# YeLyuUT/VOSDetectron

Hardware: AMD Instinct MI355X
Metric: frames/sec @1333x800 e2e_mask_rcnn_R-50-FPN, 1/2/4/8 MI355X; RoIAlign HBM GB/s (higher is better)
Workload: dtype fp32; 1 GPU; e2e_mask_rcnn_R-50-FPN_1x inference, 64 synthetic 800x1333 frames per GPU per step: blob, body, RPN, proposals, box head, class NMS, mask head -> class-selected masks (segm_results paste/RLE excluded, SURVEY 8d); frames_per_gpu_step=64, global_batch=64, layout=nhwc, gather_bytes_per_rank=0, launch=hipGraph replay per step

## Files before the change

### include/vosdet.h

```cpp
#ifndef VOSDET_H_
#define VOSDET_H_

#include <stddef.h>
#include <stdint.h>

#ifdef __cplusplus
extern "C" {
#endif

#define VD_MAX_LEVELS 5

enum {
    VD_OK = 0,
    VD_ERR_ARG = 1,
    VD_ERR_SHAPE = 2,
    VD_ERR_LAUNCH = 3,
    VD_ERR_WORKSPACE = 4
};

enum { VD_LAYOUT_NCHW = 0, VD_LAYOUT_NHWC = 1 };

#define VD_COUNT_SELECT_FAILED (-1)
#define VD_COUNT_PREV_BOXES (-2)

// ... 65 lines not shown
                        const float *bias, int relu, float *Y, void *stream);

int vd_conv3x3_wino_weight(const float *w, int Cout, int Cin, float *U, void *stream);
int vd_conv3x3_wino_bias_act(const float *X, int N, int H, int W, int C, const float *U,
                             int Cout, const float *bias, int relu, float *Y, void *stream);

int vd_conv3x3_wino4_weight(const float *w, int Cout, int Cin, float *U, void *stream);
int vd_conv3x3_wino4_bias_act(const float *X, int N, int H, int W, int C, const float *U,
                              int Cout, const float *bias, int relu, float *Y, void *stream);
int vd_conv3x3_wino4_mosaic_bias_act(const float *X, int N, int H, int W, int C, const float *U,
                                     int Cout, const float *bias, int relu, float *Y,
                                     void *stream);
int vd_conv3x3_wino4_rows_bias_act(const float *X, int N, int H, int W, int C, const float *U,
                                   int Cout, const float *bias, int relu, float *Y,
                                   void *stream);
int vd_conv3x3_wino4_grouped_bias_act(const float *X, int N, int H, int W, int C,
                                      const float *U, int groups, const float *bias, int relu,
                                      float *Y, int rows, void *stream);
int vd_conv3x3_wino4_dilated2_bias_act(const float *X, int N, int H, int W, int C,
                                       const float *U, int Cout, const float *bias, int relu,
                                       float *Y, int layout, void *stream);
int vd_conv3x3_wino4_grid_bias_act(const float *X, int N, int H, int W, int C, const float *U,
                                   int Cout, const float *bias, int relu, float *Y,
                                   void *stream);

int vd_conv3x3_wino_seg_bias_act(const float *X, int H, int W, int C, const float *U, int Cout,
                                 const float *bias, int relu, int seg_h, float *Y, void *stream);

int vd_conv3x3_wino_mosaic_bias_act(const float *X, int R, int H, int W, int C, const float *U,
                                    int Cout, const float *bias, int relu, float *Y, void *stream);
// ... 185 lines not shown
```

### vosdetectron_amd/_lib.py

```python
from __future__ import annotations

import ctypes
import os
import threading

_HERE = os.path.dirname(os.path.abspath(__file__))
LIB_PATH = os.path.join(_HERE, "libvosdet.so")
if os.environ.get("VOSDET_RESEARCH_LIB"):
    LIB_PATH = os.environ["VOSDET_RESEARCH_LIB"]
GEMM_PLANS = os.path.join(_HERE, "gemm_plans.txt")
os.environ.setdefault("VOSDET_GEMM_PLANS", GEMM_PLANS)

VD_OK, VD_ERR_ARG, VD_ERR_SHAPE, VD_ERR_LAUNCH, VD_ERR_WORKSPACE = range(5)
VD_LAYOUT_NCHW, VD_LAYOUT_NHWC = 0, 1
VD_MAX_LEVELS = 5
VD_ACT_NONE, VD_ACT_RELU, VD_ACT_SIGMOID, VD_ACT_TANH = range(4)

_lock = threading.Lock()
_lib = None


class VdFeatLevel(ctypes.Structure):
    _fields_ = [("data", ctypes.c_void_p), ("H", ctypes.c_int), ("W", ctypes.c_int),
                ("spatial_scale", ctypes.c_float)]
# ... 29 lines not shown
    "vd_gemm_dual_bias_act": (_I, [_P, _I, _P, _I, _I, _P, _I, _P, _I, _P, _P]),
    "vd_gemm_split3_weight_size": (_S, [_I, _I]),
    "vd_mask_head_upconv_logits": (_I, [_P, _I, _I, _P, _P, _P, _P, _P, _I, _P, _P]),
    "vd_gemm_split3_weight": (_I, [_P, _I, _I, _P, _P]),
    "vd_gemm_split3_bias_act": (_I, [_P, _I, _I, _P, _I, _P, _P, _I, _P, _P, _I, _I, _I, _I,
                                    _I, _P, _I, _P]),
    "vd_fpn_lateral_weight": (_I, [_P, _I, _I, _P, _P]),
    "vd_fpn_lateral_topdown": (_I, [_P, _L, _I, _P, _I, _P, _P, _I, _I, _P, _P]),
    "vd_conv3x3_bias_act": (_I, [_P, _I, _I, _I, _I, _P, _I, _P, _I, _P, _P]),
    "vd_conv3x3_wino_weight": (_I, [_P, _I, _I, _P, _P]),
    "vd_conv3x3_wino_bias_act": (_I, [_P, _I, _I, _I, _I, _P, _I, _P, _I, _P, _P]),
    "vd_conv3x3_wino4_weight": (_I, [_P, _I, _I, _P, _P]),
    "vd_conv3x3_wino4_bias_act": (_I, [_P, _I, _I, _I, _I, _P, _I, _P, _I, _P, _P]),
    "vd_conv3x3_wino4_mosaic_bias_act": (_I, [_P, _I, _I, _I, _I, _P, _I, _P, _I, _P, _P]),
    "vd_conv3x3_wino4_rows_bias_act": (_I, [_P, _I, _I, _I, _I, _P, _I, _P, _I, _P, _P]),
    "vd_conv3x3_wino4_grid_bias_act": (_I, [_P, _I, _I, _I, _I, _P, _I, _P, _I, _P, _P]),
    "vd_conv3x3_wino4_dilated2_bias_act": (_I, [_P, _I, _I, _I, _I, _P, _I, _P, _I, _P, _I,
                                                _P]),
    "vd_conv3x3_wino4_grouped_bias_act": (_I, [_P, _I, _I, _I, _I, _P, _I, _P, _I, _P, _I,
                                               _P]),
    "vd_conv3x3_wino_seg_bias_act": (_I, [_P, _I, _I, _I, _P, _I, _P, _I, _I, _P, _P]),
    "vd_conv3x3_wino_mosaic_bias_act": (_I, [_P, _I, _I, _I, _I, _P, _I, _P, _I, _P, _P]),
    "vd_roi_align_legacy_forward": (_I, [_I, _I, _F, _P, _I, _I, _I, _I, _P, _I, _P, _P]),
    "vd_roi_pool_forward": (_I, [_I, _I, _F, _P, _I, _I, _I, _I, _P, _I, _P, _P, _P]),
    "vd_roi_pool_backward": (_I, [_P, _P, _L, _P, _P]),
    "vd_roi_crop_forward": (_I, [_P, _I, _I, _I, _I, _P, _I, _I, _I, _P, _P]),
    "vd_nms_workspace_size": (_S, [_I]),
    "vd_nms": (_I, [_P, _I, _I, _F, _P, _P, _P, _S, _P]),
    "vd_map_rois_to_fpn_levels": (_I, [_P, _I, _I, _I, _I, _I, _F, _F, _P, _P]),
    "vd_mask_rois": (_I, [_P, _P, _P, _I, _I, _P, _I, _I, _I, _I, _F, _F, _P, _P, _P, _P, _P]),
# ... 77 lines not shown
```

### vosdetectron_amd/csrc/capi.cpp

```cpp
#include <hip/hip_runtime.h>

#include "vosdet_internal.hpp"

using namespace vd;

#define VD_STREAM(s) reinterpret_cast<hipStream_t>(s)

extern "C" {

int vd_version(void) { return 1; }

const char *vd_status_string(int status) {
    switch (status) {
        case VD_OK: return "ok";
        case VD_ERR_ARG: return "invalid argument";
        case VD_ERR_SHAPE: return "unsupported shape";
        case VD_ERR_LAUNCH: return "kernel launch failed";
        case VD_ERR_WORKSPACE: return "workspace too small";
        default: return "unknown status";
    }
}

static bool bad_feat(const void *p, int B, int C, int H, int W) {
    return !p || B < 1 || C < 1 || H < 1 || W < 1;
// ... 163 lines not shown

int vd_conv3x3_wino4_mosaic_bias_act(const float *X, int N, int H, int W, int C, const float *U,
                                     int Cout, const float *bias, int relu, float *Y,
                                     void *stream) {
    if (N < 0 || H < 1 || W < 1 || C < 1 || Cout < 1 || !U || !Y || (N > 0 && !X))
        return VD_ERR_ARG;
    return launch_conv3x3_wino4(X, N, H, W, C, U, Cout, bias, relu, Y, VD_STREAM(stream), 1);
}

int vd_conv3x3_wino4_rows_bias_act(const float *X, int N, int H, int W, int C, const float *U,
                                   int Cout, const float *bias, int relu, float *Y,
                                   void *stream) {
    if (N < 0 || H < 1 || W < 1 || C < 1 || Cout < 1 || !U || !Y || (N > 0 && !X))
        return VD_ERR_ARG;
    return launch_conv3x3_wino4(X, N, H, W, C, U, Cout, bias, relu, Y, VD_STREAM(stream), 2);
}

int vd_conv3x3_wino4_grouped_bias_act(const float *X, int N, int H, int W, int C,
                                      const float *U, int groups, const float *bias, int relu,
                                      float *Y, int rows, void *stream) {
    if (N < 0 || H < 1 || W < 1 || C < 1 || groups < 1 || !U || !Y || (N > 0 && !X))
        return VD_ERR_ARG;
    return launch_conv3x3_wino4(X, N, H, W, C, U, C, bias, relu, Y, VD_STREAM(stream),
                                rows ? 2 : 0, groups);
}

int vd_conv3x3_wino4_dilated2_bias_act(const float *X, int N, int H, int W, int C,
                                       const float *U, int Cout, const float *bias, int relu,
                                       float *Y, int layout, void *stream) {
    if (N < 0 || H < 2 || W < 2 || (H & 1) || (W & 1) || C < 1 || Cout < 1 || !U || !Y ||
// ... 522 lines not shown
```

### vosdetectron_amd/csrc/conv3x3_wino4.hip

```cpp
#include <stdlib.h>

#include "common.hpp"
#include "vosdet_internal.hpp"

namespace vd {

namespace {

typedef float f4v __attribute__((ext_vector_type(4)));
typedef float f2v __attribute__((ext_vector_type(2)));

constexpr int k4Co = 64;
constexpr int k4KC = 8;
constexpr int k4Threads = 512;
constexpr int k4TR = 4, k4TC = 8;
constexpr int k4PR = 4 * k4TR + 2;
constexpr int k4PC = 4 * k4TC + 2;
constexpr int k4RP = 84;
constexpr int k4PSlots = 1536;
constexpr int k4PStageB = k4PSlots * 16;
constexpr int k4VStageB = 36 * 32 * k4KC * 4;
constexpr int k4ZeroF4 = 1024;
constexpr int k4LdsB = 2 * k4VStageB + 2 * k4PStageB + 6 * 256 * 4;

// ... 49 lines not shown
    y[5] = w4_pfma(4.f, x[1], w4_pfma(-5.f, x[3], x[5]));
}

__device__ __forceinline__ void w4_at6(const float (&m)[6], float (&y)[4]) {
    const float s12 = m[1] + m[2], d12 = m[1] - m[2], s34 = m[3] + m[4], d34 = m[3] - m[4];
    y[0] = m[0] + s12 + s34;
    y[1] = __builtin_fmaf(2.f, d34, d12);
    y[2] = __builtin_fmaf(4.f, s34, s12);
    y[3] = __builtin_fmaf(8.f, d34, d12) + m[5];
}

constexpr int kStampWg = 512, kStampCh0 = 8, kStampNch = 4;
__device__ unsigned long long g_wino4_stamps[kStampWg * 8 * kStampNch * 6];

template <bool RELU, int PROBE, bool ACC = false, int VD = 1, bool STAMP = false, bool IL = false,
          bool PK = false>
__global__ __launch_bounds__(k4Threads) void conv3x3_wino4_kernel(
    const float *__restrict__ X, int N, int H, int W, int C, const float *__restrict__ U,
    int Cout, const float *__restrict__ bias, float *__restrict__ Y, int tby, int tbx,
    int cb_per_xcd, int probe_hi, int mos, int gin) {
    __shared__ __attribute__((aligned(16))) char w4_lds[k4LdsB];
    float *const vst = reinterpret_cast<float *>(w4_lds);
    char *const pst = w4_lds + 2 * k4VStageB;
    const int tid = threadIdx.x, lane = tid & 63;
    const int wave = __builtin_amdgcn_readfirstlane(tid >> 6);
    const int ncb = Cout / k4Co;
    int cb, sp;
    if (cb_per_xcd) {
        const int xcd = blockIdx.x & 7;
        cb = xcd % ncb;
        sp = (blockIdx.x >> 3) * (8 / ncb) + xcd / ncb;
    } else {
        const int r8 = blockIdx.x % (8 * ncb);
        cb = r8 / 8;
        sp = (blockIdx.x / (8 * ncb)) * 8 + (r8 & 7);
    }
    const bool pair = mos == 1, oct = mos == 3, grid = (mos & 3) == 2;
    const int hp = (mos & 3) == 0 ? mos >> 2 : 0;
    const int gG = grid ? mos >> 2 : 0, gPh = H + 1, gPw = W + 1;
    if (sp >= (pair ? (N + 1) >> 1 : oct ? (N + 7) >> 3 : ((hp || grid) ? tby * tbx : N * tby * tbx))) return;
    const int n = pair ? 2 * sp : oct ? 8 * sp : ((hp || grid) ? 0 : sp / (tby * tbx));
    const int rem = (pair || oct) ? 0 : sp - n * tby * tbx;
    const int tyb = rem / tbx, txb = rem - (rem / tbx) * tbx;
    const int oy0 = 4 * k4TR * tyb, ox0 = 4 * k4TC * txb;
    const int iy0 = oy0 - 1, ix0 = ox0 - 1;
    const int nch = ((gin & 1) ? 64 : C) / k4KC;
    const uint32_t pbase = (uint32_t)(uintptr_t)pst;

    const bool pph = (gin & 2) != 0;
    const int pNr = N >> 2;
    const float *const Xn = X + (pph ? 0 : (int64_t)n * H * W * C) + ((gin & 1) ? 64 * cb : 0);
    auto px_off = [&](int m, int y, int x) -> int64_t {
        if (pph) {
            const int ab = m / pNr, nr = m - ab * pNr;
            return (((int64_t)nr * 2 * H + 2 * y + (ab >> 1)) * (2 * W) + 2 * x + (ab & 1));
        }
        return ((int64_t)m * H + y) * W + x;
    };
    uint32_t *const poff = reinterpret_cast<uint32_t *>(pst + 2 * k4PStageB) + tid;
    constexpr int kDW = ACC ? 8 : 4;
    constexpr int kDK = 24 / kDW;
    constexpr int kPS = ACC ? 512 : 256;
    const float *const zero = reinterpret_cast<const float *>(g_wino4_zero);
    const float *srcp[kDK];
#pragma unroll
    for (int k = 0; k < kDK; ++k) {
        if (!ACC && wave >= 4) break;
        const int s = 64 * (wave + kDW * k) + lane;
        const int R = s / k4RP, u = s - R * k4RP;
        const int m = u / 5, r5 = u - 5 * m;
        const int Cc = 2 * m + (r5 >> 1), hf = r5 & 1;
        const int y = iy0 + R, x = ix0 + Cc;
        const int gx = (grid && x >= 0) ? x / gPw : 0, gy = (grid && y >= 0) ? y / gPh : 0;
        const int cell = pair ? (x >> 4) : oct ? (x >> 3) : grid ? gx : 0;
        const int xm = pair ? (x & 15) : oct ? (x & 7) : grid ? x - gx * gPw : x;
        const int mr = (hp && y >= 0) ? y / hp : (oct && y >= 0) ? 4 * (y >> 3) : grid ? gG * gy : 0;
        const int ly = hp ? y - mr * hp : oct ? (y & 7) : grid ? y - gy * gPh : y;
        const bool ok = R < k4PR && r5 < 4 && Cc < k4PC && (unsigned)ly < (unsigned)H &&
                        y >= 0 && x >= 0 && (unsigned)xm < (unsigned)W && n + cell + mr < N &&
                        (!oct || (cell < 4 && mr < 8)) && (!grid || gx < gG);
        const int64_t po = pph ? px_off(n + cell + mr, ly, xm) : px_off(cell + mr, ly, xm);
        poff[kPS * k] = ok ? (uint32_t)(po * C + 4 * hf)
                           : 0x80000000u | (uint32_t)(4 * hf);
        srcp[k] = ok ? Xn + po * C + 4 * hf : zero + 4 * hf;
    }
    auto dma = [&](int ch, int stage) {
        if constexpr (ACC) {
#pragma unroll
            for (int k = 0; k < kDK; ++k)
                w4_dma_1k(srcp[k] + ch * k4KC,
                          pbase + (uint32_t)(stage * k4PStageB + (wave + kDW * k) * 1024));
            return;
        }
        uint32_t oo[kDK];
#pragma unroll
        for (int k = 0; k < kDK; ++k) oo[k] = poff[kPS * k];
#pragma unroll
        for (int k = 0; k < kDK; ++k) {
            const uint32_t o = oo[k];
            const float *src = (o & 0x80000000u) ? zero + (o & 7u) : Xn + o + ch * k4KC;
            if (ACC && ch < 0) src = zero;
            w4_dma_1k(src, pbase + (uint32_t)(stage * k4PStageB + (wave + kDW * k) * 1024));
        }
    };

    const int ttc = lane >> 3, tci = lane & 7;
    const float *const tread =
        reinterpret_cast<const float *>(pst) + ((4 * wave) * k4RP + 10 * ttc + (tci >> 2)) * 4 +
        (tci & 3);
    const int wtile_j = 8 * (wave & 1) + ttc;
    float *const twrite =
        ACC ? vst + (wave >> 1) * 128 + 32 * (tci >> 1) + ((2 * wtile_j + (tci & 1)) ^ (8 * (tci >> 1)))
            : vst + 64 * wave + lane;
    auto transform = [&](int stage) {
        const float *tp = tread + stage * (k4PStageB / 4);
        float *vp = twrite + stage * (k4VStageB / 4);
        if (PK) {
            f2v t[6][3];
#pragma unroll
            for (int c = 0; c < 6; c += 2) {
                f2v x[6], y[6];
#pragma unroll
                for (int r = 0; r < 6; ++r)
                    x[r] = f2v{tp[(r * k4RP + 2 * c + (c >> 1)) * 4],
                               tp[(r * k4RP + 2 * (c + 1) + ((c + 1) >> 1)) * 4]};
                w4_bt6v(x, y);
#pragma unroll
                for (int a = 0; a < 6; ++a) t[a][c >> 1] = y[a];
            }
#pragma unroll
            for (int a = 0; a < 6; a += 2) {
                f2v x[6], y[6];
#pragma unroll
                for (int c = 0; c < 6; ++c)
                    x[c] = f2v{t[a][c >> 1][c & 1], t[a + 1][c >> 1][c & 1]};
                w4_bt6v(x, y);
#pragma unroll
                for (int b = 0; b < 6; ++b) {
                    vp[(6 * a + b) * 256] = y[b][0];
                    vp[(6 * (a + 1) + b) * 256] = y[b][1];
                }
            }
            return;
        }
        float t[6][6];
#pragma unroll
        for (int c = 0; c < 6; ++c) {
            float x[6], y[6];
#pragma unroll
            for (int r = 0; r < 6; ++r) x[r] = tp[(r * k4RP + 2 * c + (c >> 1)) * 4];
            w4_bt6(x, y);
#pragma unroll
            for (int a = 0; a < 6; ++a) t[a][c] = y[a];
        }
#pragma unroll
        for (int a = 0; a < 6; ++a) {
            float y[6];
            w4_bt6(t[a], y);
#pragma unroll
            for (int b = 0; b < 6; ++b) vp[(6 * a + b) * 256] = y[b];
        }
    };

    const int tg = wave >> 2, cg = wave & 3;
    const int j = lane & 15, q = lane >> 4;
// ... 18 lines not shown
        w4_uload_asm(r, ursv, (uint32_t)uvoff,
                     (uint32_t)__builtin_amdgcn_readfirstlane((ch * 4 * 18 + pos) * 1024));
    };
    f4v acc[36];
#pragma unroll
    for (int p = 0; p < 36; ++p) acc[p] = f4v{0.f, 0.f, 0.f, 0.f};
    constexpr int kUR = 9;
    f4v u[kUR];
    auto mfma_chunk = [&](bool xon, int stage, int ch, int chn, int tstage) {
        const f2v *vp = vread + stage * (k4VStageB / 8);
        const float *tpi = tread + tstage * (k4PStageB / 4);
        float *vpw = twrite + tstage * (k4VStageB / 4);
        float xc[6], tt[6][6];
        if (IL && xon) {
#pragma unroll
            for (int r = 0; r < 6; ++r) xc[r] = tpi[(r * k4RP) * 4];
        }
        if (!IL && xon) {
            if (probe_hi & 2) asm volatile("s_setprio 1" ::: "memory");
            transform(tstage);
            if (probe_hi & 2) asm volatile("s_setprio 0" ::: "memory");
        }
        f2v vq[VD][2];
#pragma unroll
        for (int d = 0; d < VD; ++d) {
            vq[d][0] = vp[(2 * d) * 128];
            vq[d][1] = vp[(2 * d + 1) * 128];
        }
        f2v b0 = vq[0][0], b1 = vq[0][1];
#pragma unroll
        for (int pp = 0; pp < 18; ++pp) {
// ... 27 lines not shown
            } else if constexpr (!(PROBE & 8)) {
                if (pp + kUR < 18)
                    u[pp % kUR] = uload(ch, pp + kUR);
                else
                    u[pp % kUR] = uload(chn, pp + kUR - 18);
            }
            if constexpr (IL) {
                if (xon && pp < 6) {
                    float y[6];
                    w4_bt6(xc, y);
#pragma unroll
                    for (int a = 0; a < 6; ++a) tt[a][pp] = y[a];
                    if (pp < 5) {
                        const int c = pp + 1;
#pragma unroll
                        for (int r = 0; r < 6; ++r) xc[r] = tpi[(r * k4RP + 2 * c + (c >> 1)) * 4];
                    }
                } else if (xon && pp < 12) {
                    const int a = pp - 6;
                    float y[6];
                    w4_bt6(tt[a], y);
#pragma unroll
                    for (int b = 0; b < 6; ++b) vpw[(6 * a + b) * 256] = y[b];
                }
            }
            __builtin_amdgcn_sched_barrier(0);
            if (pp + VD < 18) {
                vq[pp % VD][0] = n0;
                vq[pp % VD][1] = n1;
            }
            if (pp < 17) {
// ... 53 lines not shown
    asm volatile("s_waitcnt vmcnt(0)" ::: "memory");
    __syncthreads();
    if (wave < 4) transform(0);
    if (wave < 4 && nch > 1) dma(1, 1);
    asm volatile("s_waitcnt vmcnt(0)" ::: "memory");
    __syncthreads();
    for (int ch = 0; ch < nch; ++ch) {
        const int sv = ch & 1;
        const int chn = ch + 1 < nch ? ch + 1 : ch;
        if (!(PROBE & 4) && wave < 4 && ch + 2 < nch) dma(ch + 2, sv);
        mfma_chunk(!(PROBE & 1) && wave < 4 && ch + 1 < nch, sv, ch, chn, sv ^ 1);
        asm volatile("s_waitcnt vmcnt(9)" ::: "memory");
        __syncthreads();
    }
    }
    asm volatile("s_waitcnt vmcnt(0)" ::: "memory");

    const int tile = 16 * tg + j, tr = tile >> 3, tc = tile & 7;
    const int co = cb * k4Co + 16 * cg + 4 * q;
    const float4 bv = bias ? *reinterpret_cast<const float4 *>(bias + co)
                           : make_float4(0.f, 0.f, 0.f, 0.f);
    float o[16][4];
#pragma unroll
    for (int r = 0; r < 4; ++r) {
        float tt[4][6];
#pragma unroll
        for (int b = 0; b < 6; ++b) {
            float m[6], y[4];
#pragma unroll
            for (int a = 0; a < 6; ++a) m[a] = acc[6 * a + b][r];
            w4_at6(m, y);
#pragma unroll
            for (int i = 0; i < 4; ++i) tt[i][b] = y[i];
        }
#pragma unroll
        for (int i = 0; i < 4; ++i) {
            float y[4];
            w4_at6(tt[i], y);
#pragma unroll
            for (int k = 0; k < 4; ++k) o[4 * i + k][r] = y[k];
        }
    }
#pragma unroll
    for (int i = 0; i < 4; ++i) {
        const int yv = oy0 + 4 * tr + i;
        const int gy = grid ? yv / gPh : 0;
        const int mr = hp ? yv / hp : oct ? 4 * (yv >> 3) : grid ? gG * gy : 0;
        const int yy = hp ? yv - mr * hp : oct ? (yv & 7) : grid ? yv - gy * gPh : yv;
        if (yy >= H || n + mr >= N) continue;
#pragma unroll
        for (int k = 0; k < 4; ++k) {
            const int xc = ox0 + 4 * tc + k;
            const int gx = grid ? xc / gPw : 0;
            const int ncell = pair ? n + (xc >> 4) : oct ? n + mr + (xc >> 3) : n + mr + gx;
            const int xx = pair ? (xc & 15) : oct ? (xc & 7) : grid ? xc - gx * gPw : xc;
            if (xx >= W || ncell >= N || (grid && gx >= gG)) continue;
            float4 v = make_float4(o[4 * i + k][0] + bv.x, o[4 * i + k][1] + bv.y,
                                   o[4 * i + k][2] + bv.z, o[4 * i + k][3] + bv.w);
            if (RELU) {
                v.x = fmaxf(v.x, 0.f);
                v.y = fmaxf(v.y, 0.f);
                v.z = fmaxf(v.z, 0.f);
                v.w = fmaxf(v.w, 0.f);
            }
            if (!(probe_hi & 1) || v.x == 1234.5678f)
                *reinterpret_cast<float4 *>(Y + px_off(ncell, yy, xx) * Cout + co) = v;
        }
    }
// ... 279 lines not shown
bool conv3x3_wino4_supported(int C, int Cout) {
    return C % k4KC == 0 && C >= k4KC && C <= 4 * k4ZeroF4 && Cout % k4Co == 0 && Cout >= k4Co;
}

size_t conv3x3_wino4_weight_floats(int Cout, int C) { return (size_t)Cout * C * 36; }

int launch_conv3x3_wino4_weight(const float *w, int Cout, int C, float *U, hipStream_t s) {
    const int64_t n = (int64_t)Cout * C;
    if (n == 0) return VD_OK;
    if (!conv3x3_wino4_supported(C, Cout)) return VD_ERR_SHAPE;
    hipLaunchKernelGGL(wino4_weight_kernel, dim3((unsigned)((n + 255) / 256)), dim3(256), 0, s, w,
                       Cout, C, U);
    return hipGetLastError() == hipSuccess ? VD_OK : VD_ERR_LAUNCH;
}

int launch_conv3x3_wino4(const float *X, int N, int H, int W, int C, const float *U, int Cout,
                         const float *bias, int relu, float *Y, hipStream_t s, int mos,
                         int groups) {
    if ((int64_t)N * H * W == 0) return VD_OK;
    if (!conv3x3_wino4_supported(C, Cout)) return VD_ERR_SHAPE;
    int gin = groups > 1;
    if (groups == -2) {
        if (N % 4 || mos == 2 || (int64_t)N * H * W * (C > Cout ? C : Cout) >=
                                                 ((int64_t)1 << 31))
            return VD_ERR_SHAPE;
        gin = 2;
    } else if (gin && (groups < 1 || C != Cout || C % 64 || C % groups ||
                       64 % (C / groups) || mos == 1 || mos == 4)) {
        return VD_ERR_SHAPE;
    }
    if ((int64_t)N * H * W * C >= ((int64_t)1 << 40) || (int64_t)H * W * C >= ((int64_t)1 << 31))
        return VD_ERR_SHAPE;
    if (mos == 1 && (H > 15 || W > 15 || (int64_t)2 * H * W * C >= ((int64_t)1 << 31)))
        return VD_ERR_SHAPE;
    if (mos == 1 && H <= 7 && W <= 7) mos = 3;
    if (mos == 3 && (int64_t)8 * H * W * C >= ((int64_t)1 << 31)) return VD_ERR_SHAPE;
    const int hp = (H + 1 + 3) / 4 * 4;
    if (mos == 2) {
        if ((int64_t)N * H * W * C >= ((int64_t)1 << 31) || (int64_t)N * hp >= ((int64_t)1 << 30))
            return VD_ERR_SHAPE;
        mos = hp << 2;
    }
    int gG = 0;
    if (mos == 4) {
        if ((int64_t)N * H * W * C >= ((int64_t)1 << 31) || H > 255 || W > 255) return VD_ERR_SHAPE;
        int64_t best = -1;
        for (int g = 1; g <= 64 && g <= N; ++g) {
            const int64_t rows = (int64_t)(N + g - 1) / g * (H + 1);
            const int64_t b = (rows + 4 * k4TR - 1) / (4 * k4TR) *
                              (((int64_t)g * (W + 1) + 4 * k4TC - 1) / (4 * k4TC));
            if (best < 0 || b < best) best = b, gG = g;
        }
        if ((int64_t)(N + gG - 1) / gG * (H + 1) >= ((int64_t)1 << 30)) return VD_ERR_SHAPE;
    }
    const bool cells = mos == 1 || mos == 3;
    const int tby = cells ? 1
                    : gG ? (int)(((int64_t)(N + gG - 1) / gG * (H + 1) + 4 * k4TR - 1) / (4 * k4TR))
                         : ((mos ? N * hp : H) + 4 * k4TR - 1) / (4 * k4TR);
    const int tbx = cells ? 1 : ((gG ? gG * (W + 1) : W) + 4 * k4TC - 1) / (4 * k4TC);
    if (gG) mos = (gG << 2) | 2;
    const int64_t nsp = mos == 1 ? ((int64_t)N + 1) / 2
                                 : mos == 3 ? ((int64_t)N + 7) / 8
                                            : (int64_t)(mos ? 1 : N) * tby * tbx;
    const int ncb = Cout / k4Co;
    const char *cbxe = getenv("VOSDET_WINO4_CBX");
    const int cbx = (8 % ncb == 0) && !(cbxe && cbxe[0] == '0');
    const int64_t blocks = cbx ? (nsp + 8 / ncb - 1) / (8 / ncb) * 8 : (nsp + 7) / 8 * 8 * ncb;
    if (blocks > 0x7fffffff) return VD_ERR_SHAPE;
    static_assert(k4LdsB <= VD_LDS_BYTES, "LDS");
    static const int probe = [] {
        const char *e = getenv("VOSDET_WINO4_PROBE");
        return e ? atoi(e) & 15 : 0;
    }();
    static const int probe_hi = [] {
        const char *e = getenv("VOSDET_WINO4_PROBE");
        return e ? (atoi(e) >> 4) & 1 : 0;
    }();
    typedef void (*kern_t)(const float *, int, int, int, int, const float *, int, const float *,
                           float *, int, int, int, int, int, int);
    static const kern_t table[2][16] = {
        {conv3x3_wino4_kernel<false, 0>, conv3x3_wino4_kernel<false, 1>,
         conv3x3_wino4_kernel<false, 2>, conv3x3_wino4_kernel<false, 3>,
         conv3x3_wino4_kernel<false, 4>, conv3x3_wino4_kernel<false, 5>,
         conv3x3_wino4_kernel<false, 6>, conv3x3_wino4_kernel<false, 7>,
         conv3x3_wino4_kernel<false, 8>, conv3x3_wino4_kernel<false, 9>,
         conv3x3_wino4_kernel<false, 10>, conv3x3_wino4_kernel<false, 11>,
         conv3x3_wino4_kernel<false, 12>, conv3x3_wino4_kernel<false, 13>,
         conv3x3_wino4_kernel<false, 14>, conv3x3_wino4_kernel<false, 15>},
        {conv3x3_wino4_kernel<true, 0>, conv3x3_wino4_kernel<true, 1>,
         conv3x3_wino4_kernel<true, 2>, conv3x3_wino4_kernel<true, 3>,
         conv3x3_wino4_kernel<true, 4>, conv3x3_wino4_kernel<true, 5>,
         conv3x3_wino4_kernel<true, 6>, conv3x3_wino4_kernel<true, 7>,
         conv3x3_wino4_kernel<true, 8>, conv3x3_wino4_kernel<true, 9>,
         conv3x3_wino4_kernel<true, 10>, conv3x3_wino4_kernel<true, 11>,
         conv3x3_wino4_kernel<true, 12>, conv3x3_wino4_kernel<true, 13>,
         conv3x3_wino4_kernel<true, 14>, conv3x3_wino4_kernel<true, 15>}};
    const char *pse = getenv("VOSDET_WINO4_PS");
    const bool ps = pse && pse[0] == '1';
    if (ps && !probe && !mos && !gin) {
        typedef void (*kps_t)(const float *, int, int, int, int, const float *, int,
                              const float *, float *, int, int, int);
        const char *ppe = getenv("VOSDET_WINO4_PSPROBE");
        const int pp = ppe ? atoi(ppe) : 0;
#define VD_PSK(P) (relu ? conv3x3_wino4ps_kernel<true, P> : conv3x3_wino4ps_kernel<false, P>)
        kps_t kp = VD_PSK(0);
        if (pp == 1) kp = VD_PSK(1);
        if (pp == 2) kp = VD_PSK(2);
        if (pp == 4) kp = VD_PSK(4);
        if (pp == 8) kp = VD_PSK(8);
        if (pp == 16) kp = VD_PSK(16);
        if (pp == 18) kp = VD_PSK(18);
        if (pp == 31) kp = VD_PSK(31);
        if (pp == 5) kp = VD_PSK(5);
        if (pp == 12) kp = VD_PSK(12);
#undef VD_PSK
        hipLaunchKernelGGL(kp, dim3((unsigned)blocks), dim3(k4Threads), 0, s, X, N, H, W, C, U,
                           Cout, bias, Y, tby, tbx, cbx);
        return hipGetLastError() == hipSuccess ? VD_OK : VD_ERR_LAUNCH;
    }
    const char *acce = getenv("VOSDET_WINO4_ACC");
    const bool acc = !(acce && acce[0] == '0');
    const char *vde = getenv("VOSDET_WINO4_VD");
    const int vd = vde ? atoi(vde) : 1;
    const char *pke = getenv("VOSDET_WINO4_PK");
    const bool pk = !(pke && pke[0] == '0');
    kern_t kacc = relu ? conv3x3_wino4_kernel<true, 0, true, 1> : conv3x3_wino4_kernel<false, 0, true, 1>;
    if (pk)
        kacc = relu ? conv3x3_wino4_kernel<true, 0, true, 1, false, false, true>
                    : conv3x3_wino4_kernel<false, 0, true, 1, false, false, true>;
    if (vd == 2)
        kacc = relu ? conv3x3_wino4_kernel<true, 0, true, 2> : conv3x3_wino4_kernel<false, 0, true, 2>;
    if (vd == 3)
        kacc = relu ? conv3x3_wino4_kernel<true, 0, true, 3> : conv3x3_wino4_kernel<false, 0, true, 3>;
    const char *pre = getenv("VOSDET_WINO4_PRIO");
    const int prio = (pre && pre[0] == '1') ? 2 : 0;
    const char *ste = getenv("VOSDET_WINO4_STAMP");
    if (ste && ste[0] == '1')
        kacc = relu ? conv3x3_wino4_kernel<true, 0, true, 1, true>
                    : conv3x3_wino4_kernel<false, 0, true, 1, true>;
    const char *ile = getenv("VOSDET_WINO4_IL");
    if (ile && ile[0] == '1')
        kacc = relu ? conv3x3_wino4_kernel<true, 0, true, 1, false, true>
                    : conv3x3_wino4_kernel<false, 0, true, 1, false, true>;
    if (ile && ile[0] == '2')
        kacc = relu ? conv3x3_wino4_kernel<true, 0, true, 1, true, true>
                    : conv3x3_wino4_kernel<false, 0, true, 1, true, true>;
    const kern_t kern = (acc && !probe) ? kacc : table[relu ? 1 : 0][probe];
    hipLaunchKernelGGL(kern, dim3((unsigned)blocks), dim3(k4Threads), 0, s, X, N, H, W, C, U,
                       Cout, bias, Y, tby, tbx, cbx, probe_hi | prio, mos, gin);
    return hipGetLastError() == hipSuccess ? VD_OK : VD_ERR_LAUNCH;
}

}

extern "C" int vd_research_wino4_stamps(unsigned long long *host, int n) {
    const int cap = vd::kStampWg * 8 * vd::kStampNch * 6;
    if (n > cap) n = cap;
    return hipMemcpyFromSymbol(host, HIP_SYMBOL(vd::g_wino4_stamps), (size_t)n * 8, 0,
                               hipMemcpyDeviceToHost) == hipSuccess ? 0 : -1;
}
```

### vosdetectron_amd/csrc/vosdet_internal.hpp

```cpp
#pragma once

#include <hip/hip_runtime.h>
#include <stdint.h>

#include "../../include/vosdet.h"

namespace vd {

struct FpnLevels {
    const float *feat[VD_MAX_LEVELS];
    int H[VD_MAX_LEVELS];
    int W[VD_MAX_LEVELS];
    float scale[VD_MAX_LEVELS];
    int L;
    int B;
    int R;
};

int zero_async(void *p, size_t bytes, hipStream_t s);

int launch_roi_align_fwd_nchw(const float *feat, int B, int C, int H, int W, const float *rois,
                              int R, int PH, int PW, float scale, int sr, float *out,
                              hipStream_t s);
int launch_roi_align_bwd_nchw(const float *top_diff, int B, int C, int H, int W,
// ... 32 lines not shown
                       int sub_w, int relu, float *D, int cfg, hipStream_t s,
                       const float *a_bias = nullptr);
int launch_gemm_split3_mask_logits(const float *A, int M, int K, const void *Wp, int N,
                                   const float *bias, const float *cls_w, const float *cls_b,
                                   const int32_t *roi_ch, int P, float *masks, hipStream_t s);
bool gemm1x1_mfma_supported(int K, int N);
bool conv3x3_mfma_supported(int C, int Cout);
int launch_conv3x3_mfma(const float *X, int N, int H, int W, int C, const float *W2, int Cout,
                        const float *bias, int relu, float *Y, hipStream_t s);
bool conv3x3_wino_supported(int C, int Cout);
bool conv3x3_wino4_supported(int C, int Cout);
int launch_conv3x3_wino4_weight(const float *w, int Cout, int C, float *U, hipStream_t s);
int launch_conv3x3_wino4(const float *X, int N, int H, int W, int C, const float *U, int Cout,
                         const float *bias, int relu, float *Y, hipStream_t s, int mos = 0,
                         int groups = 1);
int launch_conv3x3_wino_weight(const float *w, int Cout, int C, float *U, hipStream_t s);
int launch_conv3x3_wino(const float *X, int N, int H, int W, int C, const float *U, int Cout,
                        const float *bias, int relu, float *Y, hipStream_t s, int seg_h = 0);
int launch_conv3x3_wino_mosaic(const float *X, int R, int H, int W, int C, const float *U,
                               int Cout, const float *bias, int relu, float *Y, hipStream_t s);
bool gemm1x1_dual_supported(int K1, int K2, int N);
int launch_gemm1x1_dual(const float *A1, int K1, const float *A2, int K2, int M, const float *W,
                        int N, const float *bias, int relu, float *D, hipStream_t s);
int launch_gemm1x1_mfma(const float *A, int M, int K, const float *W, int N, const float *bias,
                        const float *R, int relu, float *D, hipStream_t s);
bool fpn_lateral_supported(int K, int N);
int launch_fpn_lateral_weight(const float *W, int N, int K, float *Wf, hipStream_t s);
int launch_fpn_lateral(const float *A, int64_t M, int K, const float *Wf, int N, const float *bias,
                       const float *T, int H, int Wd, float *D, hipStream_t s);

// ... 128 lines not shown
```

### vosdetectron_amd/ops.py

```python
from __future__ import annotations

import ctypes
import os
import sys
import weakref
from typing import Optional, Sequence

import numpy as np
import torch

from . import _lib
from ._lib import VD_ERR_SHAPE, check, lib


def _stream() -> int:
    return torch.cuda.current_stream().cuda_stream


def _need(t: torch.Tensor, name: str, dtype=torch.float32) -> torch.Tensor:
    if not isinstance(t, torch.Tensor):
        raise TypeError("%s must be a torch.Tensor" % name)
    if not t.is_cuda:
        raise ValueError("%s must be a device (HIP) tensor; there is no CPU path" % name)
    if t.dtype != dtype:
# ... 734 lines not shown
    if out is None:
        out = torch.empty((N, Cout, H, W), dtype=torch.float32, device=x.device,
                          memory_format=torch.channels_last)
    fn = {False: lib().vd_conv3x3_wino4_bias_act, True: lib().vd_conv3x3_wino4_mosaic_bias_act,
          "pair": lib().vd_conv3x3_wino4_mosaic_bias_act,
          "rows": lib().vd_conv3x3_wino4_rows_bias_act,
          "grid": lib().vd_conv3x3_wino4_grid_bias_act}[mosaic]
    st = fn(x.data_ptr(), N, H, W, C, u_.data_ptr(), Cout,
            b_.data_ptr() if b_ is not None else None, int(relu), out.data_ptr(), _stream())
    if st == VD_ERR_SHAPE:
        return None
    check(st, "vd_conv3x3_wino4_bias_act (mosaic %r)" % (mosaic,))
    return out


def conv3x3_wino4_dilated2_bias_act(x: torch.Tensor, u: torch.Tensor,
                                    bias: Optional[torch.Tensor], relu: bool = False,
                                    out: Optional[torch.Tensor] = None, layout=False):
    if not x.is_cuda or x.dtype != torch.float32 or x.dim() != 4 \
            or not x.is_contiguous(memory_format=torch.channels_last):
        raise ValueError("x must be a channels_last fp32 device tensor")
    lay = {False: 0, None: 0, "pair": 1, True: 1, "grid": 2}.get(layout)
    if lay is None:
        return None
    u_ = _need(u, "u")
    N, C, H, W = x.shape
    if u_.dim() != 6 or tuple(u_.shape[1:]) != (C // 8, 4, 18, 64, 4) or C % 8 or H % 2 or W % 2:
        return None
    Cout = u_.shape[0] * 64
    b_ = _need(bias, "bias") if bias is not None else None
# ... 764 lines not shown
```

Measured before the change: 472.4 frames/s.

## Add tall tile shape and wave-quantization planner for Winograd-4 conv launches

```diff
diff --git a/include/vosdet.h b/include/vosdet.h
--- a/include/vosdet.h
+++ b/include/vosdet.h
@@ -103,6 +103,8 @@
 int vd_conv3x3_wino4_rows_bias_act(const float *X, int N, int H, int W, int C, const float *U,
                                    int Cout, const float *bias, int relu, float *Y,
                                    void *stream);
+int vd_conv3x3_wino4_plan(int N, int H, int W, int C, int Cout, int mode, int n_cu,
+                          int out[4]);
 int vd_conv3x3_wino4_grouped_bias_act(const float *X, int N, int H, int W, int C,
                                       const float *U, int groups, const float *bias, int relu,
                                       float *Y, int rows, void *stream);
diff --git a/vosdetectron_amd/_lib.py b/vosdetectron_amd/_lib.py
--- a/vosdetectron_amd/_lib.py
+++ b/vosdetectron_amd/_lib.py
@@ -67,6 +67,7 @@
     "vd_conv3x3_wino4_bias_act": (_I, [_P, _I, _I, _I, _I, _P, _I, _P, _I, _P, _P]),
     "vd_conv3x3_wino4_mosaic_bias_act": (_I, [_P, _I, _I, _I, _I, _P, _I, _P, _I, _P, _P]),
     "vd_conv3x3_wino4_rows_bias_act": (_I, [_P, _I, _I, _I, _I, _P, _I, _P, _I, _P, _P]),
+    "vd_conv3x3_wino4_plan": (_I, [_I, _I, _I, _I, _I, _I, _I, _P]),
     "vd_conv3x3_wino4_grid_bias_act": (_I, [_P, _I, _I, _I, _I, _P, _I, _P, _I, _P, _P]),
     "vd_conv3x3_wino4_dilated2_bias_act": (_I, [_P, _I, _I, _I, _I, _P, _I, _P, _I, _P, _I,
                                                 _P]),
diff --git a/vosdetectron_amd/csrc/capi.cpp b/vosdetectron_amd/csrc/capi.cpp
--- a/vosdetectron_amd/csrc/capi.cpp
+++ b/vosdetectron_amd/csrc/capi.cpp
@@ -201,6 +201,11 @@
     if (N < 0 || H < 1 || W < 1 || C < 1 || Cout < 1 || !U || !Y || (N > 0 && !X))
         return VD_ERR_ARG;
     return launch_conv3x3_wino4(X, N, H, W, C, U, Cout, bias, relu, Y, VD_STREAM(stream), 2);
+}
+
+int vd_conv3x3_wino4_plan(int N, int H, int W, int C, int Cout, int mode, int n_cu,
+                          int out[4]) {
+    return conv3x3_wino4_plan(N, H, W, C, Cout, mode, n_cu, out);
 }
 
 int vd_conv3x3_wino4_grouped_bias_act(const float *X, int N, int H, int W, int C,
diff --git a/vosdetectron_amd/csrc/conv3x3_wino4.hip b/vosdetectron_amd/csrc/conv3x3_wino4.hip
--- a/vosdetectron_amd/csrc/conv3x3_wino4.hip
+++ b/vosdetectron_amd/csrc/conv3x3_wino4.hip
@@ -1,4 +1,5 @@
 #include <stdlib.h>
+#include <string.h>
 
 #include "common.hpp"
 #include "vosdet_internal.hpp"
@@ -87,11 +88,15 @@
 __device__ unsigned long long g_wino4_stamps[kStampWg * 8 * kStampNch * 6];
 
 template <bool RELU, int PROBE, bool ACC = false, int VD = 1, bool STAMP = false, bool IL = false,
-          bool PK = false>
+          bool PK = false, bool TALL = false>
 __global__ __launch_bounds__(k4Threads) void conv3x3_wino4_kernel(
     const float *__restrict__ X, int N, int H, int W, int C, const float *__restrict__ U,
     int Cout, const float *__restrict__ bias, float *__restrict__ Y, int tby, int tbx,
-    int cb_per_xcd, int probe_hi, int mos, int gin) {
+    int cb_per_xcd, int probe_hi, int mos, int gin, int gph, int gpw) {
+    constexpr int kTR = TALL ? 8 : k4TR, kTC = TALL ? 4 : k4TC;
+    constexpr int kPR = 4 * kTR + 2, kPC = 4 * kTC + 2, kRP = TALL ? 45 : k4RP;
+    static_assert(kPR * kRP <= k4PSlots && 2 * kPC + kPC / 2 - 1 <= kRP, "patch stage");
+    static_assert(!TALL || (ACC && PK && !PROBE && !STAMP && !IL), "TALL: default form only");
     __shared__ __attribute__((aligned(16))) char w4_lds[k4LdsB];
     float *const vst = reinterpret_cast<float *>(w4_lds);
     char *const pst = w4_lds + 2 * k4VStageB;
@@ -109,13 +114,12 @@
         sp = (blockIdx.x / (8 * ncb)) * 8 + (r8 & 7);
     }
     const bool pair = mos == 1, oct = mos == 3, grid = (mos & 3) == 2;
-    const int hp = (mos & 3) == 0 ? mos >> 2 : 0;
-    const int gG = grid ? mos >> 2 : 0, gPh = H + 1, gPw = W + 1;
-    if (sp >= (pair ? (N + 1) >> 1 : oct ? (N + 7) >> 3 : ((hp || grid) ? tby * tbx : N * tby * tbx))) return;
-    const int n = pair ? 2 * sp : oct ? 8 * sp : ((hp || grid) ? 0 : sp / (tby * tbx));
+    const int gG = grid ? mos >> 2 : 0, gPh = gph, gPw = gpw;
+    if (sp >= (pair ? (N + 1) >> 1 : oct ? (N + 7) >> 3 : (grid ? tby * tbx : N * tby * tbx))) return;
+    const int n = pair ? 2 * sp : oct ? 8 * sp : (grid ? 0 : sp / (tby * tbx));
     const int rem = (pair || oct) ? 0 : sp - n * tby * tbx;
     const int tyb = rem / tbx, txb = rem - (rem / tbx) * tbx;
-    const int oy0 = 4 * k4TR * tyb, ox0 = 4 * k4TC * txb;
+    const int oy0 = 4 * kTR * tyb, ox0 = 4 * kTC * txb;
     const int iy0 = oy0 - 1, ix0 = ox0 - 1;
     const int nch = ((gin & 1) ? 64 : C) / k4KC;
     const uint32_t pbase = (uint32_t)(uintptr_t)pst;
@@ -140,16 +144,16 @@
     for (int k = 0; k < kDK; ++k) {
         if (!ACC && wave >= 4) break;
         const int s = 64 * (wave + kDW * k) + lane;
-        const int R = s / k4RP, u = s - R * k4RP;
+        const int R = s / kRP, u = s - R * kRP;
         const int m = u / 5, r5 = u - 5 * m;
         const int Cc = 2 * m + (r5 >> 1), hf = r5 & 1;
         const int y = iy0 + R, x = ix0 + Cc;
         const int gx = (grid && x >= 0) ? x / gPw : 0, gy = (grid && y >= 0) ? y / gPh : 0;
         const int cell = pair ? (x >> 4) : oct ? (x >> 3) : grid ? gx : 0;
         const int xm = pair ? (x & 15) : oct ? (x & 7) : grid ? x - gx * gPw : x;
-        const int mr = (hp && y >= 0) ? y / hp : (oct && y >= 0) ? 4 * (y >> 3) : grid ? gG * gy : 0;
-        const int ly = hp ? y - mr * hp : oct ? (y & 7) : grid ? y - gy * gPh : y;
-        const bool ok = R < k4PR && r5 < 4 && Cc < k4PC && (unsigned)ly < (unsigned)H &&
+        const int mr = (oct && y >= 0) ? 4 * (y >> 3) : grid ? gG * gy : 0;
+        const int ly = oct ? (y & 7) : grid ? y - gy * gPh : y;
+        const bool ok = R < kPR && r5 < 4 && Cc < kPC && (unsigned)ly < (unsigned)H &&
                         y >= 0 && x >= 0 && (unsigned)xm < (unsigned)W && n + cell + mr < N &&
                         (!oct || (cell < 4 && mr < 8)) && (!grid || gx < gG);
         const int64_t po = pph ? px_off(n + cell + mr, ly, xm) : px_off(cell + mr, ly, xm);
@@ -178,8 +182,9 @@
     };
 
     const int ttc = lane >> 3, tci = lane & 7;
+    const int ttr = TALL ? 2 * wave + (ttc >> 2) : wave, ttx = TALL ? (ttc & 3) : ttc;
     const float *const tread =
-        reinterpret_cast<const float *>(pst) + ((4 * wave) * k4RP + 10 * ttc + (tci >> 2)) * 4 +
+        reinterpret_cast<const float *>(pst) + ((4 * ttr) * kRP + 10 * ttx + (tci >> 2)) * 4 +
         (tci & 3);
     const int wtile_j = 8 * (wave & 1) + ttc;
     float *const twrite =
@@ -195,8 +200,8 @@
                 f2v x[6], y[6];
 #pragma unroll
                 for (int r = 0; r < 6; ++r)
-                    x[r] = f2v{tp[(r * k4RP + 2 * c + (c >> 1)) * 4],
-                               tp[(r * k4RP + 2 * (c + 1) + ((c + 1) >> 1)) * 4]};
+                    x[r] = f2v{tp[(r * kRP + 2 * c + (c >> 1)) * 4],
+                               tp[(r * kRP + 2 * (c + 1) + ((c + 1) >> 1)) * 4]};
                 w4_bt6v(x, y);
 #pragma unroll
                 for (int a = 0; a < 6; ++a) t[a][c >> 1] = y[a];
@@ -221,7 +226,7 @@
         for (int c = 0; c < 6; ++c) {
             float x[6], y[6];
 #pragma unroll
-            for (int r = 0; r < 6; ++r) x[r] = tp[(r * k4RP + 2 * c + (c >> 1)) * 4];
+            for (int r = 0; r < 6; ++r) x[r] = tp[(r * kRP + 2 * c + (c >> 1)) * 4];
             w4_bt6(x, y);
 #pragma unroll
             for (int a = 0; a < 6; ++a) t[a][c] = y[a];
@@ -270,7 +275,7 @@
         float xc[6], tt[6][6];
         if (IL && xon) {
 #pragma unroll
-            for (int r = 0; r < 6; ++r) xc[r] = tpi[(r * k4RP) * 4];
+            for (int r = 0; r < 6; ++r) xc[r] = tpi[(r * kRP) * 4];
         }
         if (!IL && xon) {
             if (probe_hi & 2) asm volatile("s_setprio 1" ::: "memory");
@@ -328,7 +333,7 @@
                     if (pp < 5) {
                         const int c = pp + 1;
 #pragma unroll
-                        for (int r = 0; r < 6; ++r) xc[r] = tpi[(r * k4RP + 2 * c + (c >> 1)) * 4];
+                        for (int r = 0; r < 6; ++r) xc[r] = tpi[(r * kRP + 2 * c + (c >> 1)) * 4];
                     }
                 } else if (xon && pp < 12) {
                     const int a = pp - 6;
@@ -412,9 +417,14 @@
         __syncthreads();
     }
     }
-    asm volatile("s_waitcnt vmcnt(0)" ::: "memory");
-
-    const int tile = 16 * tg + j, tr = tile >> 3, tc = tile & 7;
+    asm volatile("s_waitcnt vmcnt(0)"
+                 : "+v"(u[0]), "+v"(u[1]), "+v"(u[2]), "+v"(u[3]), "+v"(u[4]), "+v"(u[5]),
+                   "+v"(u[6]), "+v"(u[7]), "+v"(u[8])
+                 :
+                 : "memory");
+
+    const int tile = 16 * tg + j;
+    const int tr = TALL ? tile >> 2 : tile >> 3, tc = TALL ? (tile & 3) : (tile & 7);
     const int co = cb * k4Co + 16 * cg + 4 * q;
     const float4 bv = bias ? *reinterpret_cast<const float4 *>(bias + co)
                            : make_float4(0.f, 0.f, 0.f, 0.f);
@@ -439,17 +449,19 @@
             for (int k = 0; k < 4; ++k) o[4 * i + k][r] = y[k];
         }
     }
+    const bool gal = grid && ((gPh | gPw) & 3) == 0;
+    const int gyt = gal ? (oy0 + 4 * tr) / gPh : 0, gxt = gal ? (ox0 + 4 * tc) / gPw : 0;
 #pragma unroll
     for (int i = 0; i < 4; ++i) {
         const int yv = oy0 + 4 * tr + i;
-        const int gy = grid ? yv / gPh : 0;
-        const int mr = hp ? yv / hp : oct ? 4 * (yv >> 3) : grid ? gG * gy : 0;
-        const int yy = hp ? yv - mr * hp : oct ? (yv & 7) : grid ? yv - gy * gPh : yv;
+        const int gy = gal ? gyt : grid ? yv / gPh : 0;
+        const int mr = oct ? 4 * (yv >> 3) : grid ? gG * gy : 0;
+        const int yy = oct ? (yv & 7) : grid ? yv - gy * gPh : yv;
         if (yy >= H || n + mr >= N) continue;
 #pragma unroll
         for (int k = 0; k < 4; ++k) {
             const int xc = ox0 + 4 * tc + k;
-            const int gx = grid ? xc / gPw : 0;
+            const int gx = gal ? gxt : grid ? xc / gPw : 0;
             const int ncell = pair ? n + (xc >> 4) : oct ? n + mr + (xc >> 3) : n + mr + gx;
             const int xx = pair ? (xc & 15) : oct ? (xc & 7) : grid ? xc - gx * gPw : xc;
             if (xx >= W || ncell >= N || (grid && gx >= gG)) continue;
@@ -759,11 +771,91 @@
     return hipGetLastError() == hipSuccess ? VD_OK : VD_ERR_LAUNCH;
 }
 
+constexpr int k4PlanMaxG = 64;
+
+int conv3x3_wino4_plan(int N, int H, int W, int C, int Cout, int mode, int n_cu, int out[4]) {
+    if (N < 1 || H < 1 || W < 1 || n_cu < 1 || mode < 0 || mode > 1 || !out) return VD_ERR_ARG;
+    if (!conv3x3_wino4_supported(C, Cout)) return VD_ERR_SHAPE;
+    const int ncb = Cout / k4Co;
+    const int hp = (H + 1 + 3) / 4 * 4, wp = (W + 1 + 3) / 4 * 4;
+    auto count = [&](int tall, int g) -> int64_t {
+        const int bh = tall ? 32 : 16, bw = tall ? 16 : 32;
+        if (!mode) return (int64_t)N * ((H + bh - 1) / bh) * ((W + bw - 1) / bw);
+        const int64_t rows = (int64_t)((N + g - 1) / g) * hp, cols = (int64_t)(g - 1) * wp + W;
+        return ((rows + bh - 1) / bh) * ((cols + bw - 1) / bw);
+    };
+    auto rounds = [&](int64_t b) { return (b * ncb + n_cu - 1) / n_cu; };
+    const int gmax = mode ? (N < k4PlanMaxG ? N : k4PlanMaxG) : 1;
+    int tall = 0, g = 1;
+    const char *e = getenv("VOSDET_WINO4_PLAN");
+    if (e && e[0]) {
+        if (!strcmp(e, "0")) {
+        } else if (!strncmp(e, "tall", 4) || !strncmp(e, "wide", 4)) {
+            tall = e[0] == 't';
+            if (e[4] == ',') {
+                char *end = nullptr;
+                const long v = strtol(e + 5, &end, 10);
+                if (end == e + 5 || *end || v < 1) return VD_ERR_ARG;
+                g = v > gmax ? gmax : (int)v;
+            } else if (e[4]) {
+                return VD_ERR_ARG;
+            }
+        } else {
+            return VD_ERR_ARG;
+        }
+    } else {
+        int64_t bb = count(0, 1), br = rounds(bb);
+        for (int t = 0; t < 2; ++t)
+            for (int c = 1; c <= gmax; ++c) {
+                const int64_t b = count(t, c), r = rounds(b);
+                if (r < br || (r == br && b < bb)) bb = b, br = r, tall = t, g = c;
+            }
+    }
+    const int64_t b = count(tall, g), r = rounds(b);
+    if (b > 0x7fffffff) return VD_ERR_SHAPE;
+    out[0] = tall, out[1] = g, out[2] = (int)b, out[3] = (int)r;
+    return VD_OK;
+}
+
+namespace {
+int w4_num_cus() {
+    static const int n = [] {
+        int dev = 0, v = 0;
+        if (hipGetDevice(&dev) == hipSuccess &&
+            hipDeviceGetAttribute(&v, hipDeviceAttributeMultiprocessorCount, dev) == hipSuccess &&
+            v > 0)
+            return v;
+        return 256;
+    }();
+    return n;
+}
+}
+
 int launch_conv3x3_wino4(const float *X, int N, int H, int W, int C, const float *U, int Cout,
                          const float *bias, int relu, float *Y, hipStream_t s, int mos,
                          int groups) {
     if ((int64_t)N * H * W == 0) return VD_OK;
     if (!conv3x3_wino4_supported(C, Cout)) return VD_ERR_SHAPE;
+    static const int probe = [] {
+        const char *e = getenv("VOSDET_WINO4_PROBE");
+        return e ? atoi(e) & 15 : 0;
+    }();
+    static const int probe_hi = [] {
+        const char *e = getenv("VOSDET_WINO4_PROBE");
+        return e ? (atoi(e) >> 4) & 1 : 0;
+    }();
+    const char *pse = getenv("VOSDET_WINO4_PS");
+    const bool ps = pse && pse[0] == '1';
+    const char *acce = getenv("VOSDET_WINO4_ACC");
+    const bool acc = !(acce && acce[0] == '0');
+    const char *vde = getenv("VOSDET_WINO4_VD");
+    const int vd = vde ? atoi(vde) : 1;
+    const char *pke = getenv("VOSDET_WINO4_PK");
+    const bool pk = !(pke && pke[0] == '0');
+    const char *ste = getenv("VOSDET_WINO4_STAMP");
+    const char *ile = getenv("VOSDET_WINO4_IL");
+    const bool plain_form = acc && pk && !probe && !ps && vd != 2 && vd != 3 &&
+                            !(ste && ste[0] == '1') && !(ile && (ile[0] == '1' || ile[0] == '2'));
     int gin = groups > 1;
     if (groups == -2) {
         if (N % 4 || mos == 2 || (int64_t)N * H * W * (C > Cout ? C : Cout) >=
@@ -780,12 +872,18 @@
         return VD_ERR_SHAPE;
     if (mos == 1 && H <= 7 && W <= 7) mos = 3;
     if (mos == 3 && (int64_t)8 * H * W * C >= ((int64_t)1 << 31)) return VD_ERR_SHAPE;
-    const int hp = (H + 1 + 3) / 4 * 4;
-    if (mos == 2) {
-        if ((int64_t)N * H * W * C >= ((int64_t)1 << 31) || (int64_t)N * hp >= ((int64_t)1 << 30))
-            return VD_ERR_SHAPE;
-        mos = hp << 2;
-    }
+    const int hp = (H + 1 + 3) / 4 * 4, wp = (W + 1 + 3) / 4 * 4;
+    if (mos == 2 && ((int64_t)N * H * W * C >= ((int64_t)1 << 31) ||
+                     (int64_t)N * hp >= ((int64_t)1 << 30)))
+        return VD_ERR_SHAPE;
+    int tall = 0, sg = 1;
+    if (plain_form && (mos == 2 || (mos == 0 && gin != 2))) {
+        int pl[4];
+        const int st = conv3x3_wino4_plan(N, H, W, C, Cout, mos == 2, w4_num_cus(), pl);
+        if (st != VD_OK) return st;
+        tall = pl[0], sg = pl[1];
+    }
+    const int bh = tall ? 32 : 4 * k4TR, bw = tall ? 16 : 4 * k4TC;
     int gG = 0;
     if (mos == 4) {
         if ((int64_t)N * H * W * C >= ((int64_t)1 << 31) || H > 255 || W > 255) return VD_ERR_SHAPE;
@@ -799,11 +897,18 @@
         if ((int64_t)(N + gG - 1) / gG * (H + 1) >= ((int64_t)1 << 30)) return VD_ERR_SHAPE;
     }
     const bool cells = mos == 1 || mos == 3;
-    const int tby = cells ? 1
-                    : gG ? (int)(((int64_t)(N + gG - 1) / gG * (H + 1) + 4 * k4TR - 1) / (4 * k4TR))
-                         : ((mos ? N * hp : H) + 4 * k4TR - 1) / (4 * k4TR);
-    const int tbx = cells ? 1 : ((gG ? gG * (W + 1) : W) + 4 * k4TC - 1) / (4 * k4TC);
-    if (gG) mos = (gG << 2) | 2;
+    int gph = H + 1, gpw = W + 1;
+    int tby = cells ? 1 : (H + bh - 1) / bh, tbx = cells ? 1 : (W + bw - 1) / bw;
+    if (gG) {
+        tby = (int)(((int64_t)(N + gG - 1) / gG * gph + bh - 1) / bh);
+        tbx = (gG * gpw + bw - 1) / bw;
+        mos = (gG << 2) | 2;
+    } else if (mos == 2) {
+        gph = hp, gpw = wp;
+        tby = (int)(((int64_t)((N + sg - 1) / sg) * hp + bh - 1) / bh);
+        tbx = (int)(((int64_t)(sg - 1) * wp + W + bw - 1) / bw);
+        mos = (sg << 2) | 2;
+    }
     const int64_t nsp = mos == 1 ? ((int64_t)N + 1) / 2
                                  : mos == 3 ? ((int64_t)N + 7) / 8
                                             : (int64_t)(mos ? 1 : N) * tby * tbx;
@@ -813,16 +918,8 @@
     const int64_t blocks = cbx ? (nsp + 8 / ncb - 1) / (8 / ncb) * 8 : (nsp + 7) / 8 * 8 * ncb;
     if (blocks > 0x7fffffff) return VD_ERR_SHAPE;
     static_assert(k4LdsB <= VD_LDS_BYTES, "LDS");
-    static const int probe = [] {
-        const char *e = getenv("VOSDET_WINO4_PROBE");
-        return e ? atoi(e) & 15 : 0;
-    }();
-    static const int probe_hi = [] {
-        const char *e = getenv("VOSDET_WINO4_PROBE");
-        return e ? (atoi(e) >> 4) & 1 : 0;
-    }();
     typedef void (*kern_t)(const float *, int, int, int, int, const float *, int, const float *,
-                           float *, int, int, int, int, int, int);
+                           float *, int, int, int, int, int, int, int, int);
     static const kern_t table[2][16] = {
         {conv3x3_wino4_kernel<false, 0>, conv3x3_wino4_kernel<false, 1>,
          conv3x3_wino4_kernel<false, 2>, conv3x3_wino4_kernel<false, 3>,
@@ -840,8 +937,6 @@
          conv3x3_wino4_kernel<true, 10>, conv3x3_wino4_kernel<true, 11>,
          conv3x3_wino4_kernel<true, 12>, conv3x3_wino4_kernel<true, 13>,
          conv3x3_wino4_kernel<true, 14>, conv3x3_wino4_kernel<true, 15>}};
-    const char *pse = getenv("VOSDET_WINO4_PS");
-    const bool ps = pse && pse[0] == '1';
     if (ps && !probe && !mos && !gin) {
         typedef void (*kps_t)(const float *, int, int, int, int, const float *, int,
                               const float *, float *, int, int, int);
@@ -863,12 +958,6 @@
                            Cout, bias, Y, tby, tbx, cbx);
         return hipGetLastError() == hipSuccess ? VD_OK : VD_ERR_LAUNCH;
     }
-    const char *acce = getenv("VOSDET_WINO4_ACC");
-    const bool acc = !(acce && acce[0] == '0');
-    const char *vde = getenv("VOSDET_WINO4_VD");
-    const int vd = vde ? atoi(vde) : 1;
-    const char *pke = getenv("VOSDET_WINO4_PK");
-    const bool pk = !(pke && pke[0] == '0');
     kern_t kacc = relu ? conv3x3_wino4_kernel<true, 0, true, 1> : conv3x3_wino4_kernel<false, 0, true, 1>;
     if (pk)
         kacc = relu ? conv3x3_wino4_kernel<true, 0, true, 1, false, false, true>
@@ -879,20 +968,21 @@
         kacc = relu ? conv3x3_wino4_kernel<true, 0, true, 3> : conv3x3_wino4_kernel<false, 0, true, 3>;
     const char *pre = getenv("VOSDET_WINO4_PRIO");
     const int prio = (pre && pre[0] == '1') ? 2 : 0;
-    const char *ste = getenv("VOSDET_WINO4_STAMP");
     if (ste && ste[0] == '1')
         kacc = relu ? conv3x3_wino4_kernel<true, 0, true, 1, true>
                     : conv3x3_wino4_kernel<false, 0, true, 1, true>;
-    const char *ile = getenv("VOSDET_WINO4_IL");
     if (ile && ile[0] == '1')
         kacc = relu ? conv3x3_wino4_kernel<true, 0, true, 1, false, true>
                     : conv3x3_wino4_kernel<false, 0, true, 1, false, true>;
     if (ile && ile[0] == '2')
         kacc = relu ? conv3x3_wino4_kernel<true, 0, true, 1, true, true>
                     : conv3x3_wino4_kernel<false, 0, true, 1, true, true>;
+    if (tall)
+        kacc = relu ? conv3x3_wino4_kernel<true, 0, true, 1, false, false, true, true>
+                    : conv3x3_wino4_kernel<false, 0, true, 1, false, false, true, true>;
     const kern_t kern = (acc && !probe) ? kacc : table[relu ? 1 : 0][probe];
     hipLaunchKernelGGL(kern, dim3((unsigned)blocks), dim3(k4Threads), 0, s, X, N, H, W, C, U,
-                       Cout, bias, Y, tby, tbx, cbx, probe_hi | prio, mos, gin);
+                       Cout, bias, Y, tby, tbx, cbx, probe_hi | prio, mos, gin, gph, gpw);
     return hipGetLastError() == hipSuccess ? VD_OK : VD_ERR_LAUNCH;
 }
 
diff --git a/vosdetectron_amd/csrc/vosdet_internal.hpp b/vosdetectron_amd/csrc/vosdet_internal.hpp
--- a/vosdetectron_amd/csrc/vosdet_internal.hpp
+++ b/vosdetectron_amd/csrc/vosdet_internal.hpp
@@ -70,6 +70,7 @@
 int launch_conv3x3_wino4(const float *X, int N, int H, int W, int C, const float *U, int Cout,
                          const float *bias, int relu, float *Y, hipStream_t s, int mos = 0,
                          int groups = 1);
+int conv3x3_wino4_plan(int N, int H, int W, int C, int Cout, int mode, int n_cu, int out[4]);
 int launch_conv3x3_wino_weight(const float *w, int Cout, int C, float *U, hipStream_t s);
 int launch_conv3x3_wino(const float *X, int N, int H, int W, int C, const float *U, int Cout,
                         const float *bias, int relu, float *Y, hipStream_t s, int seg_h = 0);
diff --git a/vosdetectron_amd/ops.py b/vosdetectron_amd/ops.py
--- a/vosdetectron_amd/ops.py
+++ b/vosdetectron_amd/ops.py
@@ -772,6 +772,13 @@
     return out
 
 
+def conv3x3_wino4_plan(N: int, H: int, W: int, C: int, Cout: int, stacked: bool, n_cu: int):
+    out = (ctypes.c_int * 4)()
+    check(lib().vd_conv3x3_wino4_plan(int(N), int(H), int(W), int(C), int(Cout), int(bool(stacked)),
+                                      int(n_cu), out), "vd_conv3x3_wino4_plan")
+    return ("tall" if out[0] else "wide", int(out[1]), int(out[2]), int(out[3]))
+
+
 def conv3x3_wino4_dilated2_bias_act(x: torch.Tensor, u: torch.Tensor,
                                     bias: Optional[torch.Tensor], relu: bool = False,
                                     out: Optional[torch.Tensor] = None, layout=False):
```

Result: faster. 488.7 frames/s, median of 6 (+3.5%).
